# MiloszKrajewski/K4os.Compression.LZ4

Hardware: AMD Instinct MI355X
Metric: GiB/s encode+decode on batched 64 KiB blocks; bit-exact vs C# ref (higher is better)
Workload: dtype u8

## Files before the change

### k4os/compression/lz4_amd/csrc/k4lz4_capi.hip

```cpp
#include <hip/hip_runtime.h>
#include <stdint.h>
#include <stdio.h>
#include <stdlib.h>
#include <string.h>
#include <algorithm>
#include <atomic>
#include <memory>
#include <new>
#include <condition_variable>
#include <functional>
#include <map>
#include <mutex>
#include <string>
#include <thread>
#include <chrono>
#include <vector>

#include "../../../../include/k4lz4.h"
#include "k4lz4_decode.hpp"
#include "k4lz4_encode_fast.hpp"
#include "k4lz4_parse.hpp"
#include "k4lz4_pickle.hpp"
#include "k4lz4_segments.hpp"
#include "k4lz4_encode_hc.hpp"
// ... 416 lines not shown
    const bool parse_path = kind == KIND_ENCODE && level < K4LZ4_L03_HC && ctx->use_parse && ctx->accel == 1 && (!ctx->prof || parse_prof_ok || ctx->prof_stamp) &&
                            !(flags & (FLAG_SEGMENTS_OK | K4LZ4_FLAG_SEGMENTS | K4LZ4_FLAG_NO_SPLIT));
    const bool parse_seg_path = kind == KIND_ENCODE && level < K4LZ4_L03_HC && ctx->use_parse && ctx->parse_big && ctx->parse_seg && ctx->parse_inline_emit &&
                                ctx->accel == 1 && !ctx->prof && (flags & (FLAG_SEGMENTS_OK | K4LZ4_FLAG_SEGMENTS)) != 0 &&
                                !(flags & (K4LZ4_FLAG_NO_SPLIT | K4LZ4_FLAG_NO_REORDER | K4LZ4_FLAG_ALLOW_COPY));
    const bool parse_persistent = parse_path && ctx->parse_persist && ctx->parse_inline_emit && !ctx->prof && n > (int64_t)k4::PARSE_MAX_WAVES * (int64_t)ctx->cu_count &&
                                  !(flags & K4LZ4_FLAG_NO_REORDER);
    if (kind == KIND_ENCODE && level < K4LZ4_L03_HC && !(flags & (FLAG_SEGMENTS_OK | K4LZ4_FLAG_SEGMENTS | K4LZ4_FLAG_NO_SPLIT)) &&
        ctx->split_pct <= 0 && !ctx->prof && n > 16 * (int64_t)ctx->cu_count && !parse_persistent) {
        const int64_t parts = (n + 16 * (int64_t)ctx->cu_count - 1) / (16 * (int64_t)ctx->cu_count);
        chunk_max = (n + parts - 1) / parts;
    }
    if (parse_path && !parse_persistent) chunk_max = std::min<int64_t>(chunk_max, (int64_t)k4::PARSE_MAX_WAVES * (int64_t)ctx->cu_count);
    if (encode_like && level >= K4LZ4_L03_HC) {
        const int rc = launch_hc(ctx, kind == KIND_PICKLE ? ENV_PICKLE : kind == KIND_WRAP ? ENV_WRAP : ENV_NONE, src, srcOff, srcLen, dst, dstOff, dstCap, outLen, n, level, flags, stream, hostLen);
        if (rc != K4LZ4_OK || kind != KIND_ENCODE || !(flags & K4LZ4_FLAG_ALLOW_COPY)) return rc;
        for (int64_t first = 0; first < n; first += chunk_max) {
            const int64_t cnt = std::min<int64_t>(chunk_max, n - first);
            k4::BatchArgs a{};
            a.src = src; a.srcOff = srcOff + first; a.srcLen = srcLen + first;
            a.dst = dst; a.dstOff = dstOff + first; a.dstCap = dstCap + first; a.outLen = outLen + first; a.n = cnt;
            hipLaunchKernelGGL(k4::k4_allow_copy_kernel, dim3((unsigned)((cnt + 3) / 4)), dim3(256), 0, stream, a);
        }
        K4_HIP(ctx, hipGetLastError());
        return K4LZ4_OK;
    }
    bool may_cut = ctx->use_segments;
    if (may_cut && hostLen && n <= (int64_t)ctx->pickle_split_min) {
        may_cut = false;
        for (int64_t i = 0; i < n && !may_cut; i++) may_cut = (uint32_t)hostLen[i] >= ctx->seg_min;
    }
    if ((kind == KIND_PICKLE && (n > (int64_t)ctx->pickle_split_min || may_cut) && !ctx->prof) || kind == KIND_WRAP) {
        for (int64_t first = 0; first < n; first += chunk_max) {
            const int64_t cnt = std::min<int64_t>(chunk_max, n - first);
            const size_t need_meta = (size_t)cnt * 16 + 64;
            if (need_meta > ctx->d_pk_meta_cap) K4_HIP(ctx, hipStreamSynchronize(stream));
            int rc = grow(ctx, &ctx->d_pk_meta, &ctx->d_pk_meta_cap, need_meta, false);
            if (rc != K4LZ4_OK) return rc;
            uint64_t *d_encoff = (uint64_t *)ctx->d_pk_meta;
            int32_t *d_enccap = (int32_t *)(d_encoff + cnt);
            int32_t *d_enclen = d_enccap + cnt;
            k4::BatchArgs a{};
            a.src = src; a.srcOff = srcOff + first; a.srcLen = srcLen + first; a.dst = dst; a.dstOff = dstOff + first;
            a.dstCap = dstCap + first; a.outLen = outLen + first; a.n = cnt; a.level = level; a.accel = 1;
            a.flags = flags | (g_enforce32.load(std::memory_order_relaxed) ? K4LZ4_FLAG_X32 : 0);
            const int seg_ok = kind == KIND_PICKLE || may_cut ? FLAG_SEGMENTS_OK : 0;
            if (kind == KIND_PICKLE) hipLaunchKernelGGL(k4::k4_pickle_prep_kernel, dim3((unsigned)((cnt + 255) / 256)), dim3(256), 0, stream, a, d_encoff, d_enccap);
            else hipLaunchKernelGGL(k4::k4_wrap_prep_kernel, dim3((unsigned)((cnt + 255) / 256)), dim3(256), 0, stream, a, d_encoff, d_enccap);
            rc = launch_inner(ctx, KIND_ENCODE, src, srcOff + first, srcLen + first, dst, d_encoff, d_enccap, d_enclen, cnt, level,
                              (flags & (K4LZ4_FLAG_NO_REORDER | K4LZ4_FLAG_X32)) | K4LZ4_FLAG_RAW_RETURN | seg_ok, stream, nullptr, hostLen ? hostLen + first : nullptr);
            if (rc != K4LZ4_OK) return rc;
            if (kind == KIND_PICKLE) hipLaunchKernelGGL(k4::k4_pickle_finish_kernel, dim3((unsigned)((cnt + k4::PICKLE_FINISH_WAVES_PER_WG - 1) / k4::PICKLE_FINISH_WAVES_PER_WG)), dim3(64 * k4::PICKLE_FINISH_WAVES_PER_WG), 0, stream, a, d_enclen);
            else hipLaunchKernelGGL(k4::k4_wrap_finish_kernel, dim3((unsigned)((cnt + k4::WRAP_FINISH_WAVES_PER_WG - 1) / k4::WRAP_FINISH_WAVES_PER_WG)), dim3(64 * k4::WRAP_FINISH_WAVES_PER_WG), 0, stream, a, d_enclen);
            K4_HIP(ctx, hipGetLastError());
        }
        return K4LZ4_OK;
    }
    const bool reorder = n > 1 &&
                         (encode_like ? !(flags & K4LZ4_FLAG_NO_REORDER)
                                      : ((flags & K4LZ4_FLAG_REORDER) != 0 ||
                                         (kind == KIND_UNPICKLE && n > 64 && !(flags & K4LZ4_FLAG_NO_REORDER))));
    uint32_t *d_cost = nullptr, *d_order = nullptr, *d_hist = nullptr;
    if (reorder) {
        const size_t cnt_max = (size_t)std::min<int64_t>(chunk_max, n);
        const size_t hist_words = std::max<size_t>(2 * (size_t)k4::PCOST_BUCKETS, 2 * (size_t)k4::COST_BUCKETS + 16);
        const size_t need = cnt_max * 8 + hist_words * 4 + 64;
        if (need > ctx->d_sched_cap) K4_HIP(ctx, hipStreamSynchronize(stream));
        int rc = grow(ctx, &ctx->d_sched, &ctx->d_sched_cap, need, false);
        if (rc != K4LZ4_OK) return rc;
        d_hist = (uint32_t *)ctx->d_sched;
        d_cost = d_hist + hist_words;
        d_order = d_cost + cnt_max;
    }
    for (int64_t first = 0; first < n; first += chunk_max) {
        const int64_t cnt = std::min<int64_t>(chunk_max, n - first);
        k4::BatchArgs a{};
        a.src = src; a.srcOff = srcOff + first; a.srcLen = srcLen + first;
        a.dst = dst; a.dstOff = dstOff + first; a.dstCap = dstCap + first;
        a.outLen = outLen + first; a.n = cnt; a.level = level; a.accel = ctx->accel;
        a.flags = flags | (g_enforce32.load(std::memory_order_relaxed) ? K4LZ4_FLAG_X32 : 0);
        const bool hop2 = cnt <= (int64_t)ctx->hop2_max_per_cu * (int64_t)ctx->cu_count;
        a.prof = ctx->prof ? ctx->prof + k4::PROF_STRIDE * first : nullptr;
        a.status = ctx->d_status;
        if (((kind == KIND_ENCODE && !parse_path) || (K4_DEC_PACE && (kind == KIND_DECODE || kind == KIND_UNPICKLE))) && ctx->use_pace && ctx->d_pace && cnt > (int64_t)ctx->pace_min_per_cu * (int64_t)ctx->cu_count) {
            a.pace = ctx->d_pace;
            K4_HIP(ctx, hipMemsetAsync(a.pace, 0, k4::PACE_BYTES, stream));
        }
        k4::SegArgs sg{};
        bool seg = false;
        if (kind == KIND_ENCODE && (flags & (FLAG_SEGMENTS_OK | K4LZ4_FLAG_SEGMENTS)) && ctx->use_segments && !a.prof && !(flags & K4LZ4_FLAG_ALLOW_COPY)) {
            static_assert(k4::SEG_HDR_DWORDS * 4 == 256, "seg_first_of finds the header in front of the items");
            size_t max_items = (size_t)k4::SEG_MAX_ITEMS;
            if (hostLen) {
                size_t bound = 0;
                for (int64_t i = 0; i < cnt && bound < max_items; i++) {
                    const int32_t u = hostLen[first + i];
                    if (u > 0 && (uint32_t)u >= ctx->seg_min) bound += ((size_t)u + ctx->seg_target - 1) / ctx->seg_target;
                }
                max_items = std::min(max_items, std::max<size_t>(bound, 2));
            }
            const size_t o_items = 256, o_work = o_items + max_items * sizeof(k4::SegItem);
            const size_t o_blocks = o_work + max_items * 4, o_snaps = (o_blocks + (size_t)k4::SEG_MAX_BLOCKS * 4 + 255) & ~(size_t)255;
            const size_t o_tables = o_snaps + max_items * k4::SEG_SNAP_DWORDS * 4, total = o_tables + max_items * 16384;
            if (total > ctx->d_seg_cap || (size_t)cnt * 4 > ctx->d_seg_first_cap) {
                K4_HIP(ctx, hipStreamSynchronize(stream));
                K4_HIP(ctx, hipStreamSynchronize(ctx->aux2));
            }
            int rc = grow(ctx, &ctx->d_seg, &ctx->d_seg_cap, total, false);
            if (rc == K4LZ4_OK) rc = grow(ctx, &ctx->d_seg_first, &ctx->d_seg_first_cap, (size_t)cnt * 4, false);
            if (rc != K4LZ4_OK) return rc;
            sg.hdr = (k4::SegHdr *)ctx->d_seg; sg.items = (k4::SegItem *)(ctx->d_seg + o_items); sg.work = (uint32_t *)(ctx->d_seg + o_work);
            sg.blocks = (uint32_t *)(ctx->d_seg + o_blocks); sg.snaps = (uint32_t *)(ctx->d_seg + o_snaps); sg.tables = (uint32_t *)(ctx->d_seg + o_tables);
            sg.first = (int32_t *)ctx->d_seg_first;
            sg.seg_min = ctx->seg_min; sg.seg_target = ctx->seg_target; sg.seg_warm = ctx->seg_warm; sg.seg_div = ctx->seg_div; sg.seg_target_max = ctx->seg_target_max; sg.spin_max = ctx->seg_spin_max; sg.max_items = (uint32_t)max_items;
            hipLaunchKernelGGL(k4::k4_seg_plan_kernel, dim3(1), dim3(256), 0, stream, a, sg);
            a.seg_first = sg.first; a.seg_items = sg.items; a.seg_snaps = sg.snaps;
            seg = true;
        }
        auto segments_start = [&]() -> int {
            if (!seg) return K4LZ4_OK;
            K4_HIP(ctx, hipEventRecord(ctx->ev_fork, stream));
            K4_HIP(ctx, hipStreamWaitEvent(ctx->aux2, ctx->ev_fork, 0));
            hipLaunchKernelGGL(k4::k4_encode_seg_kernel, dim3((unsigned)((sg.max_items + k4::ENCODE_WAVES_PER_WG - 1) / k4::ENCODE_WAVES_PER_WG)), dim3(64 * k4::ENCODE_WAVES_PER_WG), 0, ctx->aux2, a, sg);
            K4_HIP(ctx, hipEventRecord(ctx->ev_join2, ctx->aux2));
            return K4LZ4_OK;
        };
        auto segments_join = [&]() -> int {
            if (!seg) return K4LZ4_OK;
            K4_HIP(ctx, hipStreamWaitEvent(stream, ctx->ev_join2, 0));
            hipLaunchKernelGGL(k4::k4_seg_join_kernel, dim3((unsigned)std::min<int64_t>(k4::SEG_MAX_BLOCKS, cnt)), dim3(64), 0, stream, a, sg);
            return K4LZ4_OK;
        };
        if (dd && dd->dict) {
            a.dict = dd->dict; a.dictOff = dd->off + first; a.dictLen = dd->len + first;
            a.dictMode = dd->mode ? dd->mode + first : nullptr;
        }
        if (reorder && parse_path && kind == KIND_ENCODE && ctx->parse_pcost) {
            a.cost = d_cost; a.hist = d_hist; a.order_out = d_order;
            K4_HIP(ctx, hipMemsetAsync(d_hist, 0, 2 * k4::PCOST_BUCKETS * 4, stream));
            hipLaunchKernelGGL(k4::k4_pcost_kernel, dim3((unsigned)((cnt + k4::PCOST_WAVES_PER_WG - 1) / k4::PCOST_WAVES_PER_WG)), dim3(64 * k4::PCOST_WAVES_PER_WG), 0, stream, a);
            hipLaunchKernelGGL(k4::k4_porder_kernel, dim3((unsigned)((cnt + 255) / 256)), dim3(256), 0, stream, a);
            a.order = d_order;
        }
        else if (reorder) {
            a.cost = d_cost; a.hist = d_hist; a.order_out = d_order;
            K4_HIP(ctx, hipMemsetAsync(d_hist, 0, (2 * k4::COST_BUCKETS + 16) * 4, stream));
            hipLaunchKernelGGL(k4::k4_cost_kernel, dim3((unsigned)cnt), dim3(64), 0, stream, a, encode_like ? 0 : 1,
                               kind == KIND_ENCODE && parse_path ? k4::COST_SAMPLE_PARSE : k4::COST_SAMPLE);
            const bool two_kernels = kind == KIND_ENCODE && !a.prof && cnt > 512 && !(flags & K4LZ4_FLAG_NO_SPLIT) &&
                                     cnt > 8 * (int64_t)ctx->cu_count && ctx->split_pct <= 0;
            k4::BatchArgs ao = a;
            ao.first = two_kernels ? (uint32_t)ctx->cost_pct : 0u;
            ao.total = (uint32_t)((int64_t)ctx->lds_floor_per_cu * (int64_t)ctx->cu_count);
            hipLaunchKernelGGL(k4::k4_order_kernel, dim3((unsigned)((cnt + 255) / 256)), dim3(256), 0, stream, ao, (uint32_t)lds_share(ctx, cnt));
            a.order = d_order;
            if (two_kernels) a.split = d_hist + 2 * k4::COST_BUCKETS;
        }
        const unsigned wg4 = (unsigned)((cnt + k4::DECODE_WAVES_PER_WG - 1) / k4::DECODE_WAVES_PER_WG);
        bool parse_here = kind == KIND_ENCODE && (parse_path || (parse_seg_path && (a.order || cnt == 1)));
        const bool big_ok = ctx->parse_big && ctx->parse_inline_emit;
        bool any_small = true, any_big = big_ok;
        if (parse_here && hostLen) {
            any_small = false; any_big = false;
            for (int64_t i = 0; i < cnt && !(any_small && (any_big || !big_ok)); i++) {
                const int32_t len = hostLen[first + i];
                if (len >= (int32_t)k4::PARSE_MIN_LEN && len < k4::LIMIT_64K) any_small = true;
                else if (len >= k4::LIMIT_64K && big_ok) any_big = true;
// ... 3861 lines not shown
```

### k4os/compression/lz4_amd/csrc/k4lz4_parse.hpp

```cpp
#pragma once
#include "k4lz4_encode_fast.hpp"
#include <type_traits>
#ifdef K4_PARSE_DEBUG
#include <stdio.h>
#include <stdlib.h>
#endif

namespace k4 {

#ifndef K4_PARSE_K
#define K4_PARSE_K 1
#endif

constexpr uint32_t PARSE_REC_STRIDE = 16448u;
static_assert(PARSE_REC_STRIDE >= ((uint32_t)LIMIT_64K - 1u - 6u) / 4u + 1u + 62u, "a block below LIMIT_64K has at most (LIMIT_64K - 1 - 6) / 4 sequences; a round adds at most 64 / 4 + 1");
constexpr uint32_t PARSE_MIN_LEN = 128u;
constexpr uint32_t PARSE_REST = 0xffffffffu;
constexpr uint32_t PARSE_BIG = 0xfffffffeu;
constexpr int PARSE_MAX_WAVES = 16;
constexpr int PARSE_LDS_TABLES = 9;
constexpr int PARSE_SEEN_DWORDS = 128;

constexpr int PARSE_LDS_DWORDS = 4096 * PARSE_LDS_TABLES + PARSE_SEEN_DWORDS * PARSE_MAX_WAVES + 4;

struct ParseArgs {
    uint2 *recs;
    uint32_t *meta;
    uint32_t *gtab;
    uint32_t nwg;
    uint32_t migrate;
    uint32_t inline_emit;
    uint32_t *nbig;
    uint32_t big;
    uint32_t slot_recs;
    uint32_t *queue;
};


template <int N> using ic = std::integral_constant<int, N>;
__device__ __forceinline__ unsigned long long uni64(unsigned long long v) { return ((unsigned long long)uni((uint32_t)(v >> 32)) << 32) | uni((uint32_t)v); }

__device__ __forceinline__ void shift16(uint32_t &w0, uint32_t &w1, uint32_t &w2, uint32_t &w3, uint32_t sh)
{
    if (sh == 0u) return;
    unsigned long long lo = ((unsigned long long)w1 << 32) | w0, hi = ((unsigned long long)w3 << 32) | w2;
    if (sh >= 16u) { lo = 0; hi = 0; }
    else if (sh >= 8u) { lo = sh == 8u ? hi : hi >> (8u * (sh - 8u)); hi = 0; }
    else { lo = (lo >> (8u * sh)) | (hi << (64u - 8u * sh)); hi >>= 8u * sh; }
    w0 = (uint32_t)lo; w1 = (uint32_t)(lo >> 32); w2 = (uint32_t)hi; w3 = (uint32_t)(hi >> 32);
}

__device__ __forceinline__ uint32_t ext12(uint32_t x0, uint32_t x1, uint32_t x2)
{
    const uint32_t t0 = min((uint32_t)(__ffs((int)x0) - 1), 32u);
    const uint32_t t1 = min((uint32_t)(__ffs((int)x1) - 1), 32u);
    const uint32_t t2 = min((uint32_t)(__ffs((int)x2) - 1), 32u);
    const uint32_t hi = t1 + (t1 == 32u ? t2 : 0u);
    return (t0 + (t0 == 32u ? hi : 0u)) >> 3;
}

__device__ __forceinline__ uint32_t ext28(const uint32_t *x)
{
    uint32_t acc = min((uint32_t)(__ffs((int)x[6]) - 1), 32u);
#pragma unroll
    for (int i = 5; i >= 0; i--) {
        const uint32_t t = min((uint32_t)(__ffs((int)x[i]) - 1), 32u);
        acc = t + (t == 32u ? acc : 0u);
    }
    return acc >> 3;
}

__device__ __forceinline__ void rec_store(uint2 *r, uint32_t x, uint32_t y)
{
#if defined(K4_NT_RECS) && !defined(K4_HOST_EMU)
    __builtin_nontemporal_store((((unsigned long long)y) << 32) | x, (unsigned long long *)r);
#else
    *r = make_uint2(x, y);
#endif
}
__device__ __forceinline__ uint2 rec_load(const uint2 *r)
{
#if defined(K4_NT_RECS) && !defined(K4_HOST_EMU)
    const unsigned long long v = __builtin_nontemporal_load((const unsigned long long *)r);
    return make_uint2((uint32_t)v, (uint32_t)(v >> 32));
#else
    return *r;
#endif
}

constexpr uint32_t HOP_LONG = 0x100u, HOP_LAZY = 0x200u, HOP_END = 0x400u, HOP_INVALID = 0x800u, HOP_TABMISS = 0x1000u;

struct ParseStats { uint32_t rounds, slow, groups, lazies, longs; };
constexpr int PARSE_FLUSH = -2;

struct ParseCtl {
    uint32_t *free_slots;
    uint32_t rec_cap;
    int claimed;
    bool resume;
    uint32_t c, sbase, sj, nrec, long_seen, long_rounds;
    bool test, more;
    uint32_t cut_pos;
    bool dry, stopped;
};

template <int K, bool GT, bool DRY = false, int TT = 1, bool SEG = false>
__device__ __forceinline__ uint32_t parse_block(const uint8_t *src, const uint32_t U, uint2 *recs, void *tabv, uint32_t *seen, const int lane, unsigned long long *pc = nullptr,
                                                ParseStats *stats = nullptr, ParseCtl *ctl = nullptr, SegRun *sr = nullptr)
{
    static_assert(!SEG || (TT != 1 && K == 1 && !DRY), "segments: byU32 blocks, one sub-window per round");
    typedef FastTable<TT> Table;
    static_assert(TT == 1 || K == 1, "byU32 tables: one sub-window per round");
    constexpr bool U32 = TT != 1;
    Table tab;
    tab.t = (decltype(tab.t))tabv;
    constexpr uint32_t SEEN_SHIFT = TT == 1 ? 1u : 0u;
    ParseStats st = {0u, 0u, 0u, 0u, 0u};
#define K4_ST(field, v) do { if (DRY) st.field += (v); } while (0)
#ifdef K4_PARSE_PROF
    unsigned long long pt[8] = {0, 0, 0, 0, 0, 0, 0, 0}, pn[8] = {0, 0, 0, 0, 0, 0, 0, 0}, plast = 0;
    const unsigned long long pbegin = prof_now<true>();
#define K4_PT(i) do { const unsigned long long t_ = prof_now<true>(); pt[i] += t_ - plast; plast = t_; } while (0)
#define K4_PN(i, v) (pn[i] += (v))
#define K4_TIC() const unsigned long long tic_ = (unsigned long long)__builtin_readcyclecounter()
#define K4_TOC(i) (pt[i] += (unsigned long long)__builtin_readcyclecounter() - tic_)
#else
#define K4_TIC() ((void)0)
#define K4_TOC(i) ((void)0)
#define K4_PT(i) ((void)0)
#define K4_PN(i, v) ((void)0)
#endif
#if defined(K4_PARSE_PROF) && !defined(K4_PARSE_PROF_SPLIT)
#define K4_TICA() K4_TIC()
#define K4_TOCA(i) K4_TOC(i)
#else
#define K4_TICA() ((void)0)
#define K4_TOCA(i) ((void)0)
#endif
#if defined(K4_PARSE_PROF) && defined(K4_PARSE_PROF_SPLIT)
#define K4_TICB() const unsigned long long ticb_ = (unsigned long long)__builtin_readcyclecounter()
#define K4_TOCB(i) (pt[i] += (unsigned long long)__builtin_readcyclecounter() - ticb_)
#define K4_TICC() const unsigned long long ticc_ = (unsigned long long)__builtin_readcyclecounter()
#define K4_TOCC(i) (pt[i] += (unsigned long long)__builtin_readcyclecounter() - ticc_)
#else
#define K4_TICB() ((void)0)
#define K4_TOCB(i) ((void)0)
#define K4_TICC() ((void)0)
#define K4_TOCC(i) ((void)0)
#endif
    const uint32_t mfl1 = U - (uint32_t)MFLIMIT + 1u;
    const uint32_t matchlimit = U - (uint32_t)LASTLITERALS;
    const unsigned long long me = 1ull << lane, below_me = me - 1ull;

    const bool resumed = ctl && ctl->resume;
    if (!resumed) for (int k = lane; k < 1024; k += 64) ((uint4 *)tabv)[k] = make_uint4(0u, 0u, 0u, 0u);
    for (int k = lane; k < PARSE_SEEN_DWORDS; k += 64) seen[k] = 0u;
    wave_sync();

    uint32_t cut_pos = 0xffffffffu;
    bool dry = false, cut_hit = false;
    uint32_t seg_begin = 0u;
    if (SEG) {
        const uint32_t ef = uni(sr->emit_from), sa = uni(sr->stop_at);
        seg_begin = uni(sr->begin);
        dry = ef != 0u;
        cut_pos = ef ? ef : sa;
    }
    if (SEG && !resumed && seg_begin != 0u) {
        if (lane == 0) tab.put(Table::hash(src + seg_begin), seg_begin);
        wave_sync();
    }
    uint32_t c = seg_begin + 1u;
    uint32_t sbase = seg_begin + 1u;
    bool test = false;
    uint32_t sj = 0u;
    uint32_t nrec = 0u;

    uint32_t seq[K], n0[K], n1[K], n2[K];
    uint32_t h[K], cpos[K], hop[K], ecode[K], pos[K];
    bool val[K];
    unsigned long long hmx[K], hits[K], Dm[K], Gall[K], vis[K];
    uint32_t qent[K];
    bool tent[K];
    U128u pw[K];
    uint32_t pre2 = 0u, pre2b = 0u;
#ifdef K4_PARSE_FORCE_MORE
    bool more = true;
#else
    bool more = false;
#endif
    U128u pw2;
    uint32_t ahead = 0u;
    uint32_t long_seen = 0u, long_rounds = 0u;

    auto prepare = [&]() {
        if (sj == 0u) {
#pragma unroll
            for (int k = 0; k < K; k++) {
                const uint32_t p = c + 64u * (uint32_t)k + (uint32_t)lane;
                const uint32_t a = p < U - 16u ? p : U - 16u;
                pw[k] = ld128u(src + a);
            }
            if (K == 1 && more) {
                const uint32_t p2 = c + 16u + (uint32_t)lane;
                pw2 = ld128u(src + (p2 < U - 16u ? p2 : U - 16u));
            }
            uint32_t o2 = c >= 2u ? c - 2u : 0u;
#if !defined(K4_HOST_EMU) && !defined(K4_EXP_PRE2_SCALAR)
            asm("" : "+v"(o2));
#endif
            pre2 = ld32u(src + o2);
            if (TT == 0) pre2b = ld32u(src + o2 + 4u);
#ifdef K4_PARSE_AHEAD
            {
                asm volatile("" :: "v"(ahead));
                const uint32_t pa = c + (uint32_t)K4_PARSE_AHEAD + 4u * (uint32_t)lane;
                ahead = ld32u(src + (pa < U - 4u ? pa : U - 4u));
            }
#endif
        } else {
            const uint32_t p = sbase + probe_offset(sj + (uint32_t)lane, 1u);
            const uint32_t a = p < U - 16u ? p : U - 16u;
            pw[0] = ld128u(src + a);
        }
    };
    if (resumed) {
        c = uni(ctl->c); sbase = uni(ctl->sbase); sj = uni(ctl->sj); nrec = uni(ctl->nrec); test = ctl->test; more = ctl->more;
        long_seen = uni(ctl->long_seen); long_rounds = uni(ctl->long_rounds);
        if (SEG) { cut_pos = uni(ctl->cut_pos); dry = uni(ctl->dry ? 1u : 0u) != 0u; }
    }
    prepare();
    (void)ahead;
    uint32_t mig_tick = 0u;

    auto visited = [&](auto kc, unsigned long long hk, uint32_t upto) -> unsigned long long {
        constexpr int k = decltype(kc)::value;
        const unsigned long long hb = hk & below_me;
        const int ph = hb ? 63 - (int)__clzll((long long)hb) : 0;
        const uint32_t qp = (uint32_t)__shfl((int)hop[k], ph) & 127u;
        const bool in = hb != 0ull && (uint32_t)lane < qp && (uint32_t)lane + 2u != qp;
        const bool before = (uint32_t)lane < qent[k] && !(tent[k] && (uint32_t)lane + 2u == qent[k]);
        const unsigned long long m = ballot(!in && !before && val[k]);
        return upto < 64u ? m & ((1ull << upto) - 1ull) : m;
    };

    auto round = [&](auto plain_c) -> bool {
        constexpr bool plain = decltype(plain_c)::value;
        const bool strided = plain ? false : sj != 0u;
        const uint32_t c0 = c;
        const int KK = strided ? 1 : K;
#ifdef K4_PARSE_PROF
        plast = prof_now<true>();
        K4_PN(0, 1); if (!plain) K4_PN(1, 1); if (strided) K4_PN(2, 1);
#endif
        K4_ST(rounds, 1u); K4_ST(slow, 1u);

        K4_PHASE("front");
        uint32_t cand[K];
        bool flagged[K];
        uint32_t hE2 = 0xffffffffu;
        if (test) hE2 = Table::hash_of(pre2, pre2b);
#pragma unroll
        for (int k = 0; k < K; k++) {
            if (k >= KK) { val[k] = false; h[k] = 0u; pos[k] = 0u; hop[k] = 0u; cpos[k] = 0u; ecode[k] = 0u; seq[k] = n0[k] = n1[k] = n2[k] = 0u; cand[k] = 0u; flagged[k] = false; continue; }
            uint32_t p;
            if (strided) {
                p = sbase + probe_offset(sj + (uint32_t)lane, 1u);
                const uint32_t pn = sbase + probe_offset(sj + (uint32_t)lane + 1u, 1u);
                val[k] = pn <= mfl1 && pn > p;
            } else {
                p = c0 + 64u * (uint32_t)k + (uint32_t)lane;
                val[k] = plain || p + 1u <= mfl1;
            }
            pos[k] = p;
            uint32_t w0 = pw[k].v[0], w1 = pw[k].v[1], w2 = pw[k].v[2], w3 = pw[k].v[3];
            if (!plain) shift16(w0, w1, w2, w3, p < U - 16u ? 0u : p - (U - 16u));
            seq[k] = w0; n0[k] = w1; n1[k] = w2; n2[k] = w3;
            h[k] = Table::hash_of(w0, w1);
            uint32_t cd = 0u;
            bool fl = false;
            if (val[k]) {
                cd = tab.get(h[k]);
                const uint32_t bit = h[k] >> SEEN_SHIFT;
                fl = ((atomicOr(&seen[bit >> 5], 1u << (bit & 31u)) >> (bit & 31u)) & 1u) != 0u;
            }
            if (h[k] == hE2) cd = c0 - 2u;
            cand[k] = cd;
            flagged[k] = fl;
        }
        K4_PT(0);
        U128u cw[K];
#pragma unroll
        for (int k = 0; k < K; k++) {
            if (k >= KK) { cw[k].v[0] = cw[k].v[1] = cw[k].v[2] = cw[k].v[3] = 0u; continue; }
            const uint32_t a = plain ? cand[k] : (cand[k] < U - 16u ? cand[k] : U - 16u);
            cw[k] = ld128u(src + a);
        }
        __builtin_amdgcn_wave_barrier();
#pragma unroll
        for (int k = 0; k < K; k++) if (k < KK && val[k]) seen[h[k] >> (5u + SEEN_SHIFT)] = 0u;

        K4_PT(1);
        K4_PHASE("groups");
#pragma unroll
        for (int k = 0; k < K; k++) { Dm[k] = 0ull; Gall[k] = 0ull; }
        {
            unsigned long long fl[K];
            unsigned long long any = 0ull;
#pragma unroll
            for (int k = 0; k < K; k++) { fl[k] = ballot(flagged[k]); any |= fl[k]; }
            if (any) {
#pragma unroll
                for (int k = 0; k < K; k++) {
                    while (fl[k]) {
                        K4_PN(3, 1); K4_ST(groups, 1u);
                        const int j = ctz64(fl[k]);
// ... 455 lines not shown
        K4_PT(5);
        return true;
    };
    auto handle_cut = [&]() -> bool {
        const uint32_t cut = c;
        if (lane == 0) tab.put(Table::hash(src + cut - 2u), cut - 2u);
        wave_sync();
        if (dry) {
            uint32_t *pub = sr->snap_pub;
#pragma unroll 2
            for (int k = lane; k < 4096; k += 64) pub[16 + k] = tab.get((uint32_t)k);
            wave_sync();
            agent_publish(pub, cut + 1u);
            dry = false;
            nrec = 0u;
            sr->cut = cut;
            cut_pos = uni(sr->stop_at);
            return false;
        }
        uint32_t theirs = 0u;
        const uint32_t spin_max = uni(sr->spin_max) ? uni(sr->spin_max) : SEG_SPIN_MAX;
        for (uint32_t spin = 0; spin < spin_max; spin++) {
            theirs = uni(agent_peek(sr->snap_chk));
            if (theirs != 0u) break;
            __builtin_amdgcn_s_sleep(8);
        }
        bool same = theirs == cut + 1u;
        if (same) {
            agent_acquire();
            bool differ = false;
#pragma unroll 2
            for (int k = lane; k < 4096; k += 64) {
                const uint32_t mine = tab.get((uint32_t)k), other = sr->snap_chk[16 + k];
                differ = differ || (mine != other && !(cut - mine > (uint32_t)DISTANCE_MAX && cut - other > (uint32_t)DISTANCE_MAX));
            }
            same = ballot(differ) == 0ull;
        }
        sr->stop = cut;
        if (!same && (theirs == 0u || !sr->fix)) { sr->state = 3u; return true; }
        if (!same) {
            uint32_t *fix = sr->fix;
#pragma unroll 2
            for (int k = lane; k < 4096; k += 64) fix[k] = tab.get((uint32_t)k);
            wave_sync();
        }
        sr->state = same ? 1u : 4u;
        return true;
    };
    if (ctl) ctl->stopped = false;
    const uint32_t rec_cap = ctl ? ctl->rec_cap : 0u;
    for (;;) {
        if (SEG) {
            cut_hit = uni(cut_hit ? 1u : 0u) != 0u;
            if (cut_hit) {
                cut_hit = false;
                if (handle_cut()) { ctl->stopped = true; return nrec; }
            }
            cut_pos = uni(cut_pos); nrec = uni(nrec); dry = uni(dry ? 1u : 0u) != 0u;
            c = uni(c); sbase = uni(sbase);
        }
        if (U32 && rec_cap && nrec + 64u * (uint32_t)K + 2u > rec_cap) {
            ctl->c = c; ctl->sbase = sbase; ctl->sj = sj; ctl->nrec = nrec; ctl->test = test; ctl->more = more;
            ctl->long_seen = long_seen; ctl->long_rounds = long_rounds;
            if (SEG) { ctl->cut_pos = cut_pos; ctl->dry = dry; }
            ctl->claimed = PARSE_FLUSH;
            return nrec;
        }
        if (GT && ctl && ctl->free_slots && (++mig_tick & 15u) == 0u) {
            const uint32_t fs = uni(lds_peek(ctl->free_slots));
            if (fs) {
                const uint32_t sl = (uint32_t)__ffs((int)fs) - 1u;
                uint32_t old = 0u;
                if (lane == 0) old = atomicAnd(ctl->free_slots, ~(1u << sl));
                if (uni(old) & (1u << sl)) {
                    ctl->c = c; ctl->sbase = sbase; ctl->sj = sj; ctl->nrec = nrec; ctl->test = test; ctl->more = more;
                    ctl->long_seen = long_seen; ctl->long_rounds = long_rounds;
                    if (SEG) { ctl->cut_pos = cut_pos; ctl->dry = dry; }
                    ctl->claimed = (int)sl;
                    wave_sync();
                    return nrec;
                }
            }
        }
        const bool plain = sj == 0u && c + 64u * (uint32_t)K + 28u <= U;
        if (K == 1 && plain && c + 63u <= sbase + 65u) {
            if (more && c + 108u <= U) { if (!fast_round(std::true_type{})) break; }
            else if (!fast_round(std::false_type{})) break;
        }
        else if (plain) { if (!round(std::true_type{})) break; }
        else if (!round(std::false_type{})) break;
    }
#ifdef K4_PARSE_PROF
    if (pc && lane == 0) {
        pc[0] = prof_now<true>() - pbegin;
        for (int i = 0; i < 6; i++) pc[1 + i] = pt[i];
        pc[7] = (unsigned long long)nrec | (pn[4] << 32);
        pc[11] = pn[0] | (pn[6] << 32);
        pc[12] = pn[1] | (pn[2] << 32);
        pc[13] = (pt[6] & 0xffffffffull) | (pt[7] << 32);
        pc[10] = pn[7];
        pc[14] = pn[3] | (pn[5] << 32);
    }
#endif
    if (DRY && stats) *stats = st;
#undef K4_ST
    if (SEG) {
        if (uni(dry ? 1u : 0u) != 0u) {
            agent_publish(sr->snap_pub, SEG_NONE);
            sr->state = 3u;
            ctl->stopped = true;
            nrec = 0u;
        } else {
            sr->stop = U; sr->state = 2u;
        }
    }
    return nrec;
}


struct EmitState { uint32_t op, emitted_to; };
template <bool HC = false, bool BIG = false>
__device__ __forceinline__ bool emit_records(const uint8_t *src, const uint32_t U, uint8_t *dst, const int dst_cap, const uint2 *recs, const uint32_t nseq, const int lane, EmitState &st);
__device__ __forceinline__ int emit_tail(const uint8_t *src, const uint32_t U, uint8_t *dst, const int dst_cap, const int lane, const EmitState &st);
template <bool HC = false, bool BIG = false>
__device__ __forceinline__ int emit_block(const uint8_t *src, const uint32_t U, uint8_t *dst, const int dst_cap, const uint2 *recs, const uint32_t nseq, const int lane)
{
    EmitState st = {0u, 0u};
    if (!emit_records<HC, BIG>(src, U, dst, dst_cap, recs, nseq, lane, st)) return 0;
    return emit_tail(src, U, dst, dst_cap, lane, st);
}

template <int K, int TT, bool SEG>
__device__ __forceinline__ int parse_one(const BatchArgs &a, const ParseArgs &p, uint32_t *lds, uint32_t *seen, const bool in_lds, const uint32_t wave, const uint32_t waves,
                                         const int lane, const long long b, const uint8_t *src, const int src_len, uint8_t *dst, const int cap, SegRun *sr, uint32_t *nrec_out)
{
    constexpr bool U32 = TT != 1;
    uint2 *recs = p.recs + (p.slot_recs ? (unsigned long long)blockIdx.x * waves + wave : (unsigned long long)b) * PARSE_REC_STRIDE;
    uint32_t n;
    unsigned long long *pc = nullptr;
#ifdef K4_PARSE_PROF
    if (a.prof) { pc = a.prof + PROF_STRIDE * b; prof_place<true>(pc, 8, lane); }
#endif
    uint32_t *free_slots = p.migrate ? lds + PARSE_LDS_DWORDS - 1 : nullptr;
    bool moved = false;
#ifndef K4_PARSE_PROF
    if (a.prof && !SEG) prof_place<true>(a.prof + PROF_STRIDE * b, 8, lane);
#endif
    EmitState est = {0u, 0u};
    bool room = true, started = false;
    auto write_out = [&](uint32_t cnt) {
        if (SEG && !started) { est.emitted_to = uni(sr->cut); started = true; }
        wave_sync();
        if (room && !emit_records<false, U32>(src, (uint32_t)src_len, dst, cap < 0 ? 0 : cap, recs, cnt, lane, est)) room = false;
        wave_sync();
    };
    uint32_t *gt = p.gtab + 4096ull * ((unsigned long long)blockIdx.x * PARSE_MAX_WAVES + wave);
    int tslot = in_lds ? (int)wave : -1;
    int my_slot = -1;
    ParseCtl ctl = {};
    ctl.free_slots = in_lds ? nullptr : free_slots; ctl.claimed = -1; ctl.resume = false;
    ctl.rec_cap = U32 ? PARSE_REC_STRIDE : 0u;
    for (;;) {
        if (tslot >= 0) n = parse_block<K, false, false, TT, SEG>(src, (uint32_t)src_len, recs, lds + 4096u * (uint32_t)tslot, seen, lane, pc, nullptr, (U32 || ctl.resume) ? &ctl : nullptr, sr);
        else n = parse_block<K, true, false, TT, SEG>(src, (uint32_t)src_len, recs, gt, seen, lane, pc, nullptr, &ctl, sr);
        if (U32 && ctl.claimed == PARSE_FLUSH) {
            if (p.inline_emit) write_out(n);
            if (!room) { n = 0u; break; }
            ctl.nrec = 0u; ctl.resume = true; ctl.claimed = -1;
            continue;
        }
        if (ctl.claimed >= 0) {
            moved = true;
            uint32_t *slot = lds + 4096u * (uint32_t)ctl.claimed;
#pragma unroll 4
            for (int k = lane; k < 1024; k += 64) ((uint4 *)slot)[k] = ((const uint4 *)gt)[k];
            wave_sync();
            my_slot = ctl.claimed;
            tslot = my_slot;
            ctl.resume = true; ctl.free_slots = nullptr; ctl.claimed = -1;
            continue;
        }
        break;
    }
    if (free_slots && lane == 0) {
        if (my_slot >= 0) atomicOr(free_slots, 1u << my_slot);
        else if (in_lds && !p.queue) atomicOr(free_slots, 1u << wave);
    }
#ifdef K4_PARSE_PROF
    if (a.prof) { if (lane == 0) { pc[9] = __builtin_amdgcn_s_memrealtime(); pc[15] = in_lds ? 1u : 2u; } }
#endif
    *nrec_out = n;
#ifndef K4_PARSE_PROF
    if (a.prof && !SEG) { prof_place<true>(a.prof + PROF_STRIDE * b, 12, lane); if (lane == 0) a.prof[PROF_STRIDE * b + 11] = in_lds ? 4u : (moved ? 6u : 5u); }
#endif
    int ret = 0;
    if (p.inline_emit) {
        const bool stopped = SEG && ctl.stopped;
        if (!(SEG && stopped && uni(sr->state) == 3u)) {
            if (room) write_out(n);
            if (room) ret = stopped ? (int)est.op : emit_tail(src, (uint32_t)src_len, dst, cap < 0 ? 0 : cap, lane, est);
        }
    }
#ifndef K4_PARSE_PROF
    if (a.prof && !SEG) prof_place<true>(a.prof + PROF_STRIDE * b, 9, lane);
#endif
    (void)moved;
    return ret;
}

template <int K, int TT = 1>
__device__ __forceinline__ void parse_kernel_body(const BatchArgs &a, const ParseArgs &p, uint32_t *lds)
{
    constexpr bool U32 = TT != 1;
    const int lane = lane_id();
    const uint32_t wave = uni(threadIdx.x >> 6);
    const uint32_t waves = blockDim.x >> 6;
    const uint32_t lds_tables = waves < (uint32_t)PARSE_LDS_TABLES ? waves : (uint32_t)PARSE_LDS_TABLES;
    uint32_t *seen = lds + 4096u * (uint32_t)PARSE_LDS_TABLES + (uint32_t)PARSE_SEEN_DWORDS * wave;
    const bool in_lds = wave < lds_tables;
    if (U32 && p.nbig && uni(*(volatile uint32_t *)p.nbig) == 0u) return;
    if (p.migrate) {
        if (threadIdx.x == 0) lds[PARSE_LDS_DWORDS - 1] = 0u;
        __syncthreads();
    }
    for (long long idx = (long long)wave * (long long)p.nwg + (long long)blockIdx.x;;) {
        if (p.queue) {
            uint32_t t = 0u;
            if (lane == 0) {
                t = atomicAdd(p.queue, 1u);
                if (t < (uint32_t)a.n) t = in_lds ? atomicAdd(p.queue + 1, 1u) : (uint32_t)a.n - 1u - atomicAdd(p.queue + 2, 1u);
                else t = 0xffffffffu;
            }
            t = uni(t);
            if (t == 0xffffffffu) {
                if (p.migrate && in_lds && lane == 0) atomicOr(lds + PARSE_LDS_DWORDS - 1, 1u << wave);
                return;
            }
            idx = (long long)t;
        }
        if (idx >= a.n) return;
        const long long b = a.order ? (long long)uni(a.order[idx]) : idx;
        const int src_len = a.srcLen[b];
        uint32_t *meta = p.meta + 2ull * (unsigned long long)b;
        const bool big = src_len >= LIMIT_64K && a.accel == 1;
        const bool mine = a.accel == 1 && (U32 ? big : (src_len >= (int)PARSE_MIN_LEN && src_len < LIMIT_64K));
        if (!mine) {
            if (!U32 && lane == 0) {
                meta[0] = (big && p.big) ? PARSE_BIG : PARSE_REST; meta[1] = 0u;
                if (big && p.big && p.nbig) atomicAdd(p.nbig, 1u);
            }
        } else {
            uint32_t n = 0u;
            const int ret = parse_one<K, TT, false>(a, p, lds, seen, in_lds, wave, waves, lane, b, a.src + a.srcOff[b], src_len, a.dst + a.dstOff[b], a.dstCap[b], nullptr, &n);
            if (lane == 0) {
                meta[0] = n; meta[1] = 0u;
                if (p.inline_emit) a.outLen[b] = codec_encode_result(src_len, ret, a.flags);
            }
        }
        if (!p.queue) return;
    }
}


__global__ __launch_bounds__(64 * PARSE_MAX_WAVES) void k4_parse_kernel(BatchArgs a, ParseArgs p)
{
    __shared__ __attribute__((aligned(16))) uint32_t lds[PARSE_LDS_DWORDS];
    parse_kernel_body<K4_PARSE_K>(a, p, lds);
}

__global__ __launch_bounds__(64 * PARSE_MAX_WAVES) void k4_parse_big_kernel(BatchArgs a, ParseArgs p)
{
    __shared__ __attribute__((aligned(16))) uint32_t lds[PARSE_LDS_DWORDS];
    if (a.flags & FLAG_X32) parse_kernel_body<1, 2>(a, p, lds);
    else parse_kernel_body<1, 0>(a, p, lds);
}


constexpr uint32_t PCOST_SAMPLE = 3072u;
constexpr int PCOST_BUCKETS = 512;
constexpr int PCOST_WAVES_PER_WG = 8;

__device__ __forceinline__ uint32_t pcost_bucket(unsigned long long cost)
{
    if (cost < 256ull) return 0u;
    const uint32_t l = 63u - (uint32_t)__clzll((long long)cost);
    const uint32_t b = 16u * (l - 8u) + (uint32_t)((cost >> (l - 4u)) & 15ull) + 1u;
    return b < (uint32_t)PCOST_BUCKETS ? b : (uint32_t)PCOST_BUCKETS - 1u;
}

__global__ __launch_bounds__(64 * PCOST_WAVES_PER_WG) void k4_pcost_kernel(BatchArgs a)
{
    __shared__ __attribute__((aligned(16))) uint32_t lds[PCOST_WAVES_PER_WG][4096 + PARSE_SEEN_DWORDS];
    const int lane = lane_id();
    const uint32_t wave = uni(threadIdx.x >> 6);
    const long long b = (long long)blockIdx.x * PCOST_WAVES_PER_WG + (long long)wave;
    if (b >= a.n) return;
    const int src_len = a.srcLen[b];
    unsigned long long cost = 0ull;
    if (src_len >= (int)PARSE_MIN_LEN && src_len < LIMIT_64K) {
        const uint32_t sample = (uint32_t)src_len < PCOST_SAMPLE ? (uint32_t)src_len : PCOST_SAMPLE;
        ParseStats st;
        const uint32_t nseq = parse_block<1, false, true>(a.src + a.srcOff[b], sample, nullptr, (uint16_t *)lds[wave], lds[wave] + 4096, lane, nullptr, &st);
        const unsigned long long cyc = 6500ull * st.rounds + 3000ull * st.slow + 120ull * nseq + 150ull * st.groups + 480ull * st.lazies + 1500ull * st.longs;
        cost = cyc * (unsigned long long)(uint32_t)src_len / sample;
    } else if (src_len > 0) {
        cost = 120ull * (unsigned long long)(uint32_t)src_len;
    }
    if (lane == 0) {
        const uint32_t bkt = pcost_bucket(cost);
        a.cost[b] = bkt;
        atomicAdd(&a.hist[bkt], 1u);
    }
}

__global__ __launch_bounds__(256) void k4_porder_kernel(BatchArgs a)
{
    __shared__ uint32_t before[PCOST_BUCKETS];
    for (int k = (int)threadIdx.x; k < PCOST_BUCKETS; k += 256) before[k] = a.hist[k];
    __syncthreads();
    if (threadIdx.x == 0) {
        uint32_t acc = 0u;
        for (int k = PCOST_BUCKETS - 1; k >= 0; k--) { const uint32_t c = before[k]; before[k] = acc; acc += c; }
    }
    __syncthreads();
    const long long b = (long long)blockIdx.x * 256 + threadIdx.x;
    if (b >= a.n) return;
    const uint32_t bkt = a.cost[b];
    a.order_out[before[bkt] + atomicAdd(&a.hist[PCOST_BUCKETS + bkt], 1u)] = (uint32_t)b;
}


constexpr int EMIT_WAVES_PER_WG = 4;

template <bool HC, bool BIG>
__device__ __forceinline__ bool emit_records(const uint8_t *src, const uint32_t U, uint8_t *dst, const int dst_cap, const uint2 *recs, const uint32_t nseq, const int lane, EmitState &st)
{
    const bool limited = dst_cap < compress_bound((int)U);
    const uint64_t olimit = (uint64_t)(dst_cap < 0 ? 0 : dst_cap);
    uint32_t op = st.op, emitted_to = st.emitted_to;
    uint2 rn = make_uint2(0u, 0u);
    if ((uint32_t)lane < nseq) rn = rec_load(recs + lane);
    for (uint32_t base = 0u; base < nseq; base += 64u) {
        const uint32_t n = nseq - base < 64u ? nseq - base : 64u;
        const bool mine = (uint32_t)lane < n;
        const uint2 r = rn;
        if (base + 64u + (uint32_t)lane < nseq) rn = rec_load(recs + base + 64u + (uint32_t)lane);
        const uint32_t pos = r.x, cpos = r.x - (r.y & 0xffffu);
        uint32_t code = r.y >> 16;
        if (BIG) {
// ... 153 lines not shown
```

Measured before the change: 61.62.

## Enable progress-based wave pacing priorities in the byU16 parse kernel

Extends the existing pace mechanism, previously used only by the non-parse encode path, to the parse-path encode kernel. Each wave periodically reports its parse position through Pace::update, which can raise or lower its hardware scheduling priority so lagging waves finish sooner and the tail of the batch shrinks. A per-wave LDS slot is added and a global pace buffer is cleared before each parse launch. The cost is extra periodic atomics and LDS traffic in the hot parse loop plus a memset per launch.

```diff
diff --git a/k4os/compression/lz4_amd/csrc/k4lz4_capi.hip b/k4os/compression/lz4_amd/csrc/k4lz4_capi.hip
--- a/k4os/compression/lz4_amd/csrc/k4lz4_capi.hip
+++ b/k4os/compression/lz4_amd/csrc/k4lz4_capi.hip
@@ -522,7 +522,7 @@
         const bool hop2 = cnt <= (int64_t)ctx->hop2_max_per_cu * (int64_t)ctx->cu_count;
         a.prof = ctx->prof ? ctx->prof + k4::PROF_STRIDE * first : nullptr;
         a.status = ctx->d_status;
-        if (((kind == KIND_ENCODE && !parse_path) || (K4_DEC_PACE && (kind == KIND_DECODE || kind == KIND_UNPICKLE))) && ctx->use_pace && ctx->d_pace && cnt > (int64_t)ctx->pace_min_per_cu * (int64_t)ctx->cu_count) {
+        if ((kind == KIND_ENCODE || (K4_DEC_PACE && (kind == KIND_DECODE || kind == KIND_UNPICKLE))) && ctx->use_pace && ctx->d_pace && cnt > (int64_t)ctx->pace_min_per_cu * (int64_t)ctx->cu_count) {
             a.pace = ctx->d_pace;
             K4_HIP(ctx, hipMemsetAsync(a.pace, 0, k4::PACE_BYTES, stream));
         }
diff --git a/k4os/compression/lz4_amd/csrc/k4lz4_parse.hpp b/k4os/compression/lz4_amd/csrc/k4lz4_parse.hpp
--- a/k4os/compression/lz4_amd/csrc/k4lz4_parse.hpp
+++ b/k4os/compression/lz4_amd/csrc/k4lz4_parse.hpp
@@ -10,6 +10,9 @@
 
 #ifndef K4_PARSE_K
 #define K4_PARSE_K 1
+#endif
+#ifndef K4_PARSE_PACE
+#define K4_PARSE_PACE 1
 #endif
 
 constexpr uint32_t PARSE_REC_STRIDE = 16448u;
@@ -22,6 +25,7 @@
 constexpr int PARSE_SEEN_DWORDS = 128;
 
 constexpr int PARSE_LDS_DWORDS = 4096 * PARSE_LDS_TABLES + PARSE_SEEN_DWORDS * PARSE_MAX_WAVES + 4;
+constexpr int PARSE_PACE_DWORDS = PARSE_MAX_WAVES;
 
 struct ParseArgs {
     uint2 *recs;
@@ -104,10 +108,11 @@
     bool dry, stopped;
 };
 
-template <int K, bool GT, bool DRY = false, int TT = 1, bool SEG = false>
+template <int K, bool GT, bool DRY = false, int TT = 1, bool SEG = false, bool PACE = false>
 __device__ __forceinline__ uint32_t parse_block(const uint8_t *src, const uint32_t U, uint2 *recs, void *tabv, uint32_t *seen, const int lane, unsigned long long *pc = nullptr,
-                                                ParseStats *stats = nullptr, ParseCtl *ctl = nullptr, SegRun *sr = nullptr)
-{
+                                                ParseStats *stats = nullptr, ParseCtl *ctl = nullptr, SegRun *sr = nullptr, uint32_t *pace = nullptr, uint32_t *pace_mine = nullptr)
+{
+    static_assert(!PACE || (TT == 1 && !DRY && !SEG), "priorities: the byU16 blocks of k4_parse_kernel");
     static_assert(!SEG || (TT != 1 && K == 1 && !DRY), "segments: byU32 blocks, one sub-window per round");
     typedef FastTable<TT> Table;
     static_assert(TT == 1 || K == 1, "byU32 tables: one sub-window per round");
@@ -232,6 +237,8 @@
     prepare();
     (void)ahead;
     uint32_t mig_tick = 0u;
+    uint32_t pace_c = c;
+    (void)pace_c;
 
     auto visited = [&](auto kc, unsigned long long hk, uint32_t upto) -> unsigned long long {
         constexpr int k = decltype(kc)::value;
@@ -853,6 +860,22 @@
                 }
             }
         }
+#ifndef K4_PARSE_PRIO_STATIC
+        if constexpr (PACE)
+#else
+        if constexpr (false)
+#endif
+        {
+            if (pace && ((c ^ pace_c) >> PACE_STEP_LOG2) != 0u) {
+                pace_c = c;
+                const int level = Pace::update(pace, pace_mine, c, U, lane);
+#ifndef K4_PARSE_PROF
+                if (pc && lane == 0) { const unsigned long long v = pc[13], top = v >> 32, lv = level > 0 ? (unsigned long long)level : 0ull; pc[13] = ((v & 0xffffffffull) + 1ull) | ((lv > top ? lv : top) << 32); }
+#else
+                (void)level;
+#endif
+            }
+        }
         const bool plain = sj == 0u && c + 64u * (uint32_t)K + 28u <= U;
         if (K == 1 && plain && c + 63u <= sbase + 65u) {
             if (more && c + 108u <= U) { if (!fast_round(std::true_type{})) break; }
@@ -915,8 +938,25 @@
     uint32_t *free_slots = p.migrate ? lds + PARSE_LDS_DWORDS - 1 : nullptr;
     bool moved = false;
 #ifndef K4_PARSE_PROF
-    if (a.prof && !SEG) prof_place<true>(a.prof + PROF_STRIDE * b, 8, lane);
-#endif
+    if (a.prof && !SEG) {
+        prof_place<true>(a.prof + PROF_STRIDE * b, 8, lane);
+        if (TT == 1 && lane == 0) a.prof[PROF_STRIDE * b + 14] =(unsigned long long)(1u + wave) | ((unsigned long long)blockIdx.x << 8);
+    }
+#endif
+    constexpr bool PACE = K4_PARSE_PACE && TT == 1 && !SEG;
+    uint32_t *pace_mine = nullptr;
+    if constexpr (PACE) {
+#ifndef K4_HOST_EMU
+        pace_mine = lds + PARSE_LDS_DWORDS + wave;
+#endif
+        Pace::begin(a.pace, pace_mine, lane);
+#ifdef K4_PARSE_PRIO_STATIC
+        if (a.pace) { if (in_lds) __builtin_amdgcn_s_setprio(0); else __builtin_amdgcn_s_setprio(1); }
+#endif
+#ifndef K4_PARSE_PROF
+        if (a.prof) pc = a.prof + PROF_STRIDE * b;
+#endif
+    }
     EmitState est = {0u, 0u};
     bool room = true, started = false;
     auto write_out = [&](uint32_t cnt) {
@@ -932,8 +972,8 @@
     ctl.free_slots = in_lds ? nullptr : free_slots; ctl.claimed = -1; ctl.resume = false;
     ctl.rec_cap = U32 ? PARSE_REC_STRIDE : 0u;
     for (;;) {
-        if (tslot >= 0) n = parse_block<K, false, false, TT, SEG>(src, (uint32_t)src_len, recs, lds + 4096u * (uint32_t)tslot, seen, lane, pc, nullptr, (U32 || ctl.resume) ? &ctl : nullptr, sr);
-        else n = parse_block<K, true, false, TT, SEG>(src, (uint32_t)src_len, recs, gt, seen, lane, pc, nullptr, &ctl, sr);
+        if (tslot >= 0) n = parse_block<K, false, false, TT, SEG, PACE>(src, (uint32_t)src_len, recs, lds + 4096u * (uint32_t)tslot, seen, lane, pc, nullptr, (U32 || ctl.resume) ? &ctl : nullptr, sr, a.pace, pace_mine);
+        else n = parse_block<K, true, false, TT, SEG, PACE>(src, (uint32_t)src_len, recs, gt, seen, lane, pc, nullptr, &ctl, sr, a.pace, pace_mine);
         if (U32 && ctl.claimed == PARSE_FLUSH) {
             if (p.inline_emit) write_out(n);
             if (!room) { n = 0u; break; }
@@ -946,6 +986,9 @@
 #pragma unroll 4
             for (int k = lane; k < 1024; k += 64) ((uint4 *)slot)[k] = ((const uint4 *)gt)[k];
             wave_sync();
+#ifdef K4_PARSE_PRIO_STATIC
+            if (TT == 1 && !SEG) __builtin_amdgcn_s_setprio(0);
+#endif
             my_slot = ctl.claimed;
             tslot = my_slot;
             ctl.resume = true; ctl.free_slots = nullptr; ctl.claimed = -1;
@@ -965,6 +1008,11 @@
     if (a.prof && !SEG) { prof_place<true>(a.prof + PROF_STRIDE * b, 12, lane); if (lane == 0) a.prof[PROF_STRIDE * b + 11] = in_lds ? 4u : (moved ? 6u : 5u); }
 #endif
     int ret = 0;
+#ifdef K4_PARSE_WRITEOUT_PRIO
+    if constexpr (PACE) {
+        if (a.pace) { const uint32_t pr = __builtin_amdgcn_s_getreg((1 << 11) | (3 << 6) | 2); if (pr >= 2u) __builtin_amdgcn_s_setprio(3); }
+    }
+#endif
     if (p.inline_emit) {
         const bool stopped = SEG && ctl.stopped;
         if (!(SEG && stopped && uni(sr->state) == 3u)) {
@@ -1035,7 +1083,7 @@
 
 __global__ __launch_bounds__(64 * PARSE_MAX_WAVES) void k4_parse_kernel(BatchArgs a, ParseArgs p)
 {
-    __shared__ __attribute__((aligned(16))) uint32_t lds[PARSE_LDS_DWORDS];
+    __shared__ __attribute__((aligned(16))) uint32_t lds[PARSE_LDS_DWORDS + PARSE_PACE_DWORDS];
     parse_kernel_body<K4_PARSE_K>(a, p, lds);
 }
 
```

Result: no change. 62.14, median of 6 (+0.8%).
